# dash-robotics/perception

Hardware: AMD Instinct MI355X
Metric: frames/sec (640x480 D435 cloud, plane+cluster+ICP) (higher is better)
Workload: dtype f32

## Files before the change

perception_amd/csrc/common.hpp:

```cpp
#pragma once
#include <hip/hip_runtime.h>
#include <stdint.h>

#include "../../include/cuboid_hip.h"

namespace cd {

constexpr int WAVE = 64;
constexpr int BLOCK = 256;
constexpr int WAVES_PER_BLOCK = BLOCK / WAVE;
constexpr int ITEMS = 8;
constexpr int TILE = BLOCK * ITEMS;
constexpr int WAVE_SPAN = WAVE * ITEMS;
constexpr int RADIX_BITS = 8;
constexpr int RADIX = 1 << RADIX_BITS;
#ifndef CD_SORT_BLOCK
#define CD_SORT_BLOCK 1024
#endif
constexpr int SORT_BLOCK = CD_SORT_BLOCK;
constexpr int SORT_TILE = SORT_BLOCK * ITEMS;
constexpr int KICP = CD_MAX_CLUSTERS_PER_FRAME;
constexpr int FIX_SHIFT = 32;
constexpr int FIX_SHIFT_D2 = 36;
constexpr int RND_TABLE = 1 << 15;
// ... 23 lines not shown
    int32_t n_v;
    int32_t n_plane;
    int32_t n_o;
    int32_t n_k;
    int32_t n_hyp;
    int32_t sampler_exhausted;
    int32_t ksize[KICP];
    int32_t koff[KICP];
    float origin[3];
    int32_t n_cropped;
    int32_t cl_done;
    int32_t crop_overflow;
    int32_t scan_stalled;
    int32_t n_runs;
    int32_t digit_vary;
    int32_t pad_;
};

struct CropLimits {
    float zlo, zhi, xlo, xhi;
};

struct KeyPack {
    int32_t enabled;
    int32_t bi, bj;
    int32_t ilo, jlo, klo;
};

struct BBoxGate {
    double P[12];
    float rect[4];
// ... 240 lines not shown
```

perception_amd/csrc/cuboid_hip.hip:

```cpp
#include <algorithm>
#include <cstdio>
#include <cstdlib>
#include <cstring>
#include <memory>
#include <atomic>
#include <mutex>
#include <shared_mutex>
#include <condition_variable>
#include <random>
#include <vector>

#include "device_buffer.hpp"
#include "host_math.hpp"
#include "kernels.hpp"
#include "overlay_math.hpp"
#include "texture_math.hpp"

using namespace cd;

struct cd_streams {
    hipStream_t stream = nullptr, stream2 = nullptr, stream3 = nullptr;
    hipEvent_t ev[8] = {nullptr}, ev2[3] = {nullptr, nullptr, nullptr};
    ~cd_streams() {
        for (auto& e : ev2) if (e) hipEventDestroy(e);
// ... 5 lines not shown
struct cd_context : cd_streams {
    int device = 0;
    int N = 0, F = 0, T = 0;
    char err[512] = {0};
    DevBuf<char> d_in;
    DevBuf<uint16_t> d_depth;
    DevBuf<uint8_t> d_color;
    DevBuf<FrameState> d_fs;
    PinBuf<FrameState> h_fs;
    DevBuf<int> d_tileA, d_tileB, d_tileK, d_tileC;
    bool batch_zeroed = false;
    bool crop_two_pass = false;
    int icp_persist = 1;
    DevBuf<float4> d_cpt, d_vox, d_obj, d_src0, d_src;
    DevBuf<uint32_t> d_key[2], d_val[2], d_ghist;
    DevBuf<int> d_sstate;
    DevBuf<unsigned long long> d_tile64;
    bool crop_runs = true;
    DevBuf<int> d_ticket;
    DevBuf<int> d_rnd, d_valid, d_counts, d_active, d_have;
    PinBuf<int> h_valid, h_counts, h_active, h_have;
    DevBuf<float4> d_models, d_model;
    PinBuf<float4> h_model, h_models;
    DevBuf<unsigned long long> d_sums;
    PinBuf<unsigned long long> h_sums;
    DevBuf<int> d_plane_idx, d_head, d_next, d_parent, d_csize, d_rank, d_cand, d_sizes, d_label;
    DevBuf<float4> d_tpl, d_tlo, d_thi;
    DevBuf<float4> d_tplk, d_tlok, d_thik;
    DevBuf<IcpGrid> d_grid;
    DevBuf<unsigned short> d_kdmap;
// ... 10 lines not shown
    std::vector<IcpState> st_init;
    int force_stall = 0;
    int scan_retries = 0;
    int persist_gave_up = 0;
    int n_cu = 256;
    int icp_mode = 0;
    int icp_max_wg = 0;
    int icp_cpw = 0;
    bool fs_initialised = false;
    int icp_direct = 1;
    int mirror_reads = 1;
    int mirror_writes = 1;
    int cluster_cells = 1;
    int crop_direct = 1;
    int centroid_lanes = 1;
    bool voxel_runs = true;
    int icp_slots = 0;
    int icp_big_weight = 0;
    DevBuf<int> d_order; PinBuf<int> h_order;
    int tpl_cap = 0, tpl_used = 0;
    std::shared_ptr<const struct PreparedTemplate> tpl_prep[CD_MAX_TEMPLATES];
    int tpl_off[CD_MAX_TEMPLATES] = {0}, tpl_m[CD_MAX_TEMPLATES] = {0};
    bool tpl_gridded[CD_MAX_TEMPLATES] = {false};
    bool tpl_big[CD_MAX_TEMPLATES] = {false};
    DevBuf<IcpSuper> d_super;
    DevBuf<IcpLattice> d_lat;
    int tpl_faces[CD_MAX_TEMPLATES] = {0};
    int icp_lattice = 1;
    int zero_once = 1;
    int copy_kernels = 1;
// ... 281 lines not shown
        if (!over) break;
        if (std::getenv("CUBOID_DEBUG")) std::fprintf(stderr, "cuboid_hip: single-pass crop overflowed, redoing the batch in two passes\n");
        kp.enabled = 0;
        crop_runs = false;
        for (int f = 0; f < F; ++f) {
            FrameState& s = c->h_fs[f];
            std::memset(&s, 0, sizeof(s));
            for (int a = 0; a < 3; ++a) { s.mn[a] = 0xffffffffu; s.mx[a] = 0u; }
            }
    }
    int max_nc = 0, max_bits = 0;
    for (int f = 0; f < F; ++f) { max_nc = std::max(max_nc, c->h_fs[f].n_c); max_bits = std::max(max_bits, c->h_fs[f].key_bits); }
    const int Tc = std::max(1, (max_nc + TILE - 1) / TILE);
    const int Tsc = std::max(1, (max_nc + SORT_TILE - 1) / SORT_TILE);
    const int npass = (max_bits + RADIX_BITS - 1) / RADIX_BITS;
    int cur = 0;
    const bool by_runs = c->voxel_runs && npass > 0 && c->N <= (1 << 20);
    int Tc_runs = Tc;
    uint32_t* const key[2] = {c->d_key[0], c->d_key[1]}, * const val[2] = {c->d_val[0], c->d_val[1]};
    if (crop_runs) {
        int vary = 0, max_runs = 0;
        for (int f = 0; f < F; ++f) {
            if (c->h_fs[f].n_c > 0) vary |= c->h_fs[f].digit_vary;
            max_runs = std::max(max_runs, c->h_fs[f].n_runs);
        }
        int digits[4], nd = 0;
        for (int d = 0; d < 4; ++d) if ((vary >> d) & 1) digits[nd++] = d;
        const int Tsr = std::max(1, (max_runs + SORT_TILE - 1) / SORT_TILE);
        Tc_runs = std::max(1, (max_runs + TILE - 1) / TILE);
        LAUNCH(c, cur = launch_radix_scatter_runs(c->stream, key, val, c->N, F, Tsr, digits, nd, c->d_fs, c->d_ghist, c->d_sstate, c->d_ticket));
    } else if (by_runs)
        LAUNCH(c, cur = launch_radix_sort_runs(c->stream, key, val, c->N, F, T, Tsc, npass, c->d_fs, c->d_ghist, c->d_sstate, c->d_tileA, kp, c->d_ticket));
    else
        LAUNCH(c, cur = launch_radix_sort(c->stream, key, val, c->N, F, Tsc, npass, c->d_fs, c->d_ghist, c->d_sstate, kp, c->d_ticket));
    if (cur < 0) return fail(c, CD_ERR_DEVICE, "radix sort: the scan state could not be zeroed");
    const uint32_t* vin = c->d_val[cur];
    ZERO_FILL(c, c->d_tileC, sizeof(int) * (size_t)F * T);
    if (crop_runs || by_runs)
        LAUNCH(c, launch_voxel_centroid_runs(c->stream, c->d_key[cur], vin, crop_runs && direct_pts ? reinterpret_cast<const float4*>(d_in) : c->d_cpt, c->N, F, T, crop_runs ? Tc_runs : Tc,
                                             rgb_off >= 0 ? 1 : 0, c->d_fs, c->d_tileC, c->d_vox, c->d_ticket, c->centroid_lanes, crop_runs && direct_pts ? N : c->N));
    else
        LAUNCH(c, launch_voxel_centroid(c->stream, c->d_key[cur], vin, c->d_cpt, c->N, F, T, Tc, rgb_off >= 0 ? 1 : 0, c->d_fs, c->d_tileC, c->d_vox, c->d_ticket));
    if (rounds_out) *rounds_out = 0;
    return CD_OK;
}

int stage_plane(cd_context* c, int F, const cd_params* p, std::vector<int>& iterations, int* rounds_out, const float* axes = nullptr) {
    const int T = c->T;
    const bool mr = c->mirror_reads != 0;
    const float thr = hm::fold_ge(p->plane_distance_threshold);
    int max_nv = 0;
    for (int f = 0; f < F; ++f) max_nv = std::max(max_nv, c->h_fs[f].n_v);
    const int Tv = std::max(1, (max_nv + TILE - 1) / TILE);
// ... 859 lines not shown

int zero_batch_scratch(cd_context* c, int F) {
    ZeroRegions zr;
    zr.n = 0;
    zr.fs = c->mirror_writes && c->copy_kernels ? c->d_fs : nullptr;
    zr.nfs = F;
    c->fs_initialised = zr.fs != nullptr;
    auto add = [&](void* ptr, size_t bytes) { zr.ptr[zr.n] = (uint32_t*)ptr; zr.words[zr.n] = bytes / 4; ++zr.n; };
    const size_t FT = (size_t)F * c->T;
    add(c->d_ticket, sizeof(int) * (size_t)F * TICKET_PITCH);
    add(c->d_tileA, sizeof(int) * FT);
    add(c->d_tileB, sizeof(int) * FT);
    add(c->d_tileC, sizeof(int) * FT);
    add(c->d_tile64, sizeof(unsigned long long) * FT);
    add(c->d_ghist, sizeof(uint32_t) * (size_t)F * SORT_MAX_PASSES_HOST * RADIX);
    add(c->d_counts, sizeof(int) * (size_t)F * MAX_HYP);
    add(c->d_sums, sizeof(unsigned long long) * 10 * (size_t)F);
    add(c->d_tileK, sizeof(int) * FT * KICP);
    add(c->d_acc, sizeof(unsigned long long) * 48 * (size_t)c->cl_cap);
    add(c->d_accf, sizeof(unsigned long long) * ((size_t)c->cl_cap + 1));
    add(c->d_queue, sizeof(int) * 16);
    LAUNCH(c, launch_zero_regions(c->stream, zr));
    c->batch_zeroed = true;
    return CD_OK;
}

int batch_prologue(cd_context* c, int gate_source, const void* d_frames, int F, const DepthJob* dj) {
    if (gate_source == CD_BBOX_PER_FRAME) {
        std::memcpy(c->h_rects, c->frame_rects.data(), sizeof(int32_t) * 4 * (size_t)F);
        HIPCHK(c, xfer(c, c->d_rects, c->h_rects, sizeof(int32_t) * 4 * (size_t)F, hipMemcpyHostToDevice));
// ... 328 lines not shown
    switch (which) {
        case 0: return (int)sizeof(cd_params);
        case 1: return (int)sizeof(cd_cluster_result);
        case 2: return (int)sizeof(cd_frame_result);
        case 3: return (int)sizeof(cd_timing);
        case 4: return (int)sizeof(cd_depth_camera);
        case 5: return (int)sizeof(cd_color_gate_params);
        case 6: return (int)sizeof(cd_color_bbox);
        case 7: return (int)sizeof(cd_overlay_params);
        case 8: return (int)sizeof(cd_overlay_box);
        default: return -1;
    }
}

const char* cd_last_error(const cd_context* ctx) { return ctx ? ctx->err : "null context"; }

void cd_destroy(cd_context* c) {
    if (!c) return;
    hipSetDevice(c->device);
    for (hipStream_t q : {c->stream, c->stream2, c->stream3}) if (q) hipStreamSynchronize(q);
    delete c;
}

int cd_create(int device_id, int max_points, int max_frames, cd_context** out) {
    if (!out) return CD_ERR_INVALID_ARG;
    *out = nullptr;
    if (max_points <= 0 || max_frames <= 0) return CD_ERR_INVALID_ARG;
    int ndev = 0;
    if (hipGetDeviceCount(&ndev) != hipSuccess || ndev <= 0 || device_id < 0 || device_id >= ndev) return CD_ERR_DEVICE;
    if (hipSetDevice(device_id) != hipSuccess) return CD_ERR_DEVICE;
// ... 4 lines not shown
    c->F = max_frames;
    c->T = (max_points + TILE - 1) / TILE;
    const size_t N = (size_t)c->N, F = (size_t)c->F, T = (size_t)c->T, FN = F * N;
    if (const char* m = std::getenv("CUBOID_ICP_LOWPRIO")) c->icp_lowprio = std::atoi(m);
    int prio_least = 0, prio_greatest = 0;
    if (hipDeviceGetStreamPriorityRange(&prio_least, &prio_greatest) != hipSuccess) prio_least = prio_greatest = 0;
    bool ok = hipStreamCreateWithPriority(&c->stream, hipStreamNonBlocking, 0) == hipSuccess;
    for (auto& e : c->ev) ok = ok && hipEventCreate(&e) == hipSuccess;
    ok = ok && ALLOC(d_fs, F) && ALLOC(h_fs, F);
    ok = ok && ALLOC(d_tileA, F * T) && ALLOC(d_tileB, F * T) && ALLOC(d_tileK, F * KICP * T) && ALLOC(d_tileC, F * T);
    ok = ok && ALLOC(d_cpt, FN) && ALLOC(d_vox, FN) && ALLOC(d_obj, FN);
    ok = ok && ALLOC(d_src0, FN) && ALLOC(d_src, FN);
    for (int k = 0; k < 2; ++k) ok = ok && ALLOC(d_key[k], FN) && ALLOC(d_val[k], FN);
    ok = ok && ALLOC(d_ghist, F * SORT_MAX_PASSES_HOST * RADIX);
    ok = ok && ALLOC(d_sstate, (size_t)SORT_MAX_PASSES_HOST * F * RADIX * ((N + SORT_TILE - 1) / SORT_TILE));
    ok = ok && ALLOC(d_tile64, F * T);
    ok = ok && ALLOC(d_ticket, (size_t)F * TICKET_PITCH) && hipMemset(c->d_ticket, 0, sizeof(int) * (size_t)F * TICKET_PITCH) == hipSuccess;
    ok = ok && ALLOC(d_rnd, (size_t)RND_TABLE);
    ok = ok && ALLOC(d_models, F * MAX_HYP) && ALLOC(d_valid, F * MAX_HYP) && ALLOC(d_counts, F * MAX_HYP);
    ok = ok && ALLOC(h_valid, F * MAX_HYP) && ALLOC(h_counts, F * MAX_HYP) && ALLOC(h_models, F * MAX_HYP);
    ok = ok && ALLOC(d_active, F) && ALLOC(h_active, F);
    ok = ok && ALLOC(d_model, F) && ALLOC(h_model, F);
    ok = ok && ALLOC(d_have, F) && ALLOC(h_have, F);
    ok = ok && ALLOC(d_sums, F * 10) && ALLOC(h_sums, F * 10);
    ok = ok && ALLOC(d_plane_idx, FN) && ALLOC(d_head, F * CELL_BUCKETS);
    ok = ok && ALLOC(d_next, FN) && ALLOC(d_parent, FN) && ALLOC(d_csize, FN);
    ok = ok && ALLOC(d_rank, FN) && ALLOC(d_cand, FN) && ALLOC(d_sizes, FN) && ALLOC(d_label, FN);
    c->tpl_cap = 1 << 18;
    ok = ok && ALLOC(d_tpl, (size_t)c->tpl_cap);
    ok = ok && ALLOC(d_super, (size_t)CD_MAX_TEMPLATES);
    ok = ok && ALLOC(d_lat, (size_t)CD_MAX_TEMPLATES);
// ... 17 lines not shown
    c->cl_cap = (int)ncl;
    c->work_cap = (int)(F * (N / 64 + KICP + 1));
    ok = ok && ALLOC(d_cl, ncl) && ALLOC(h_cl, ncl);
    ok = ok && ALLOC(d_order, ncl) && ALLOC(h_order, ncl);
    if (const char* m = std::getenv("CUBOID_ICP_MAX_WG")) c->icp_max_wg = std::max(0, std::atoi(m));
    if (const char* m = std::getenv("CUBOID_ICP_CPW")) c->icp_cpw = std::max(0, std::atoi(m));
    if (const char* m = std::getenv("CUBOID_ICP_SLOTS")) c->icp_slots = std::max(0, std::atoi(m));
    if (const char* m = std::getenv("CUBOID_ICP_DONATE")) c->icp_donate = std::atoi(m);
    if (const char* m = std::getenv("CUBOID_ICP_DON_IDLE")) c->don_idle = std::max(0, std::atoi(m));
    if (const char* m = std::getenv("CUBOID_ICP_DON_FAULT")) c->don_fault = std::atoi(m);
    if (const char* m = std::getenv("CUBOID_ICP_LATTICE")) c->icp_lattice = std::atoi(m);
    if (const char* m = std::getenv("CUBOID_COPY_KERNELS")) c->copy_kernels = std::atoi(m);
    if (const char* m = std::getenv("CUBOID_ZERO_ONCE")) c->zero_once = std::atoi(m);
    if (const char* m = std::getenv("CUBOID_LAT_SHAPE")) std::sscanf(m, "%d,%d,%d", &c->lat_shape[0], &c->lat_shape[1], &c->lat_shape[2]);
    if (const char* m = std::getenv("CUBOID_VOXEL_RUNS")) c->voxel_runs = std::atoi(m) != 0;
    if (const char* m = std::getenv("CUBOID_CENTROID_LANES")) c->centroid_lanes = std::atoi(m) != 0;
    if (const char* m = std::getenv("CUBOID_CROP_DIRECT")) c->crop_direct = std::atoi(m) != 0;
    if (const char* m = std::getenv("CUBOID_CLUSTER_CELLS")) c->cluster_cells = std::atoi(m) != 0;
    if (const char* m = std::getenv("CUBOID_MIRROR_WRITES")) c->mirror_writes = std::atoi(m) != 0;
    if (const char* m = std::getenv("CUBOID_MIRROR_READS")) c->mirror_reads = std::atoi(m) != 0;
    if (const char* m = std::getenv("CUBOID_ICP_DIRECT")) c->icp_direct = std::atoi(m) != 0;
    if (const char* m = std::getenv("CUBOID_ICP_BIG_WEIGHT")) c->icp_big_weight = std::max(0, std::atoi(m));
    if (const char* m = std::getenv("CUBOID_CROP_TWO_PASS")) c->crop_two_pass = std::atoi(m) != 0;
    if (const char* m = std::getenv("CUBOID_ICP_PERSIST")) c->icp_persist = std::atoi(m);
    if (const char* m = std::getenv("CUBOID_FORCE_SCAN_STALL")) c->force_stall = std::max(0, std::atoi(m));
    if (const char* m = std::getenv("CUBOID_CROP_RUNS")) c->crop_runs = std::atoi(m) != 0;
    if (const char* m = std::getenv("CUBOID_ICP_CONCURRENT")) c->icp_concurrent = std::max(0, std::atoi(m));
    if (const char* m = std::getenv("CUBOID_FRONT_CONCURRENT")) c->front_concurrent = std::max(0, std::atoi(m));
    if (const char* m = std::getenv("CUBOID_ICP_MODE")) c->icp_mode = !std::strcmp(m, "sliced") ? 1 : (!std::strcmp(m, "cluster") ? 2 : (!std::strcmp(m, "pipe") ? 3 : 0));
    ok = ok && ALLOC(d_work, (size_t)c->work_cap) && ALLOC(h_work, (size_t)c->work_cap);
// ... 1511 lines not shown
```

perception_amd/csrc/k_voxel.hip:

```cpp
#include "kernels.hpp"

namespace cd {

template <int R>
__device__ __forceinline__ void load_rows(const char* __restrict__ in, size_t stride, size_t fbase, int first, int N, int rgb_off,
                                          float (&x)[R], float (&y)[R], float (&z)[R], uint32_t (&rgb)[R]) {
    if (stride == 16 && rgb_off == 12) {
        float4 v[R];
#pragma unroll
        for (int j = 0; j < R; ++j) v[j] = *reinterpret_cast<const float4*>(in + (fbase + (size_t)min(first + j * WAVE, N - 1)) * 16);
#pragma unroll
        for (int j = 0; j < R; ++j) { x[j] = v[j].x; y[j] = v[j].y; z[j] = v[j].z; rgb[j] = __float_as_uint(v[j].w); }
    } else {
#pragma unroll
        for (int j = 0; j < R; ++j) {
            const char* p = in + (fbase + (size_t)min(first + j * WAVE, N - 1)) * stride;
            x[j] = *reinterpret_cast<const float*>(p);
            y[j] = *reinterpret_cast<const float*>(p + 4);
            z[j] = *reinterpret_cast<const float*>(p + 8);
            rgb[j] = rgb_off >= 0 ? *reinterpret_cast<const uint32_t*>(p + rgb_off) : 0u;
        }
    }
}

// ... 112 lines not shown
        const int hi = (int)floorf(__fmul_rn(mx[a], inv));
        s.min_b[a] = lo;
        s.div_b[a] = hi - lo + 1;
        cells *= (long long)(hi - lo + 1);
        if (cells > 2147483647ll) bad = true;
    }
    if (bad) { s.status = CD_ERR_LEAF_TOO_SMALL; s.n_c = 0; s.n_runs = 0; return; }
    int bits = 1;
    while (bits < 31 && (1ll << bits) < cells) ++bits;
    s.key_bits = bits;
}
__global__ void __launch_bounds__(WAVE) k_voxel_setup(FrameState* __restrict__ fs, float leaf, const uint32_t* __restrict__ ghist,
                                                      FrameState* __restrict__ mirror) {
    CD_FRONT_PRIO();
    const int f = blockIdx.x, lane = threadIdx.x;
    int vary = 0;
    if (ghist) {
        for (int d = 0; d < 4; ++d) {
            int bins = 0;
            for (int q = 0; q < RADIX / WAVE; ++q) bins += __popcll(__ballot(ghist[((size_t)f * 4 + d) * RADIX + q * WAVE + lane] != 0u));
            if (bins > 1) vary |= 1 << d;
        }
    }
    if (lane != 0) return;
    FrameState s = fs[f];
    if (ghist) s.digit_vary = vary;
    voxel_setup_frame(s, leaf);
    fs[f] = s;
    if (mirror) mirror[f] = s;
}

__global__ void __launch_bounds__(BLOCK) k_crop_compact(const char* __restrict__ in, size_t stride, int N, int pitch,
                                                        int rgb_off, CropLimits lim, int T, float leaf,
                                                        const FrameState* __restrict__ fs,
                                                        const int* __restrict__ tile_off, float4* __restrict__ cpt,
                                                        uint32_t* __restrict__ keys) {
    CD_FRONT_PRIO();
    __shared__ int s_cnt[WAVES_PER_BLOCK];
    const int f = blockIdx.y, tile = blockIdx.x, w = threadIdx.x >> 6, lane = threadIdx.x & 63;
    if (fs[f].n_c <= 0) return;
    const size_t fbase = (size_t)f * N;
// ... 501 lines not shown
            }
        }
        if (ql == 0) {
            const float c = (float)cnt;
            uint32_t packed = 0;
            if (rgb_on) {
                const int R = (int)__fdiv_rn(cr, c), G = (int)__fdiv_rn(cg, c), B = (int)__fdiv_rn(cb, c);
                packed = ((uint32_t)R << 16) | ((uint32_t)G << 8) | (uint32_t)B;
            }
            vox[fbase + out0 + h] = make_float4(__fdiv_rn(sx, c), __fdiv_rn(sy, c), __fdiv_rn(sz, c), __uint_as_float(packed));
        }
        h = hn; e0 = ne0; kk = nkk; rec = nrec; have = nhave;
    }
}

__global__ void __launch_bounds__(BLOCK) k_voxel_centroid_lanes(const uint32_t* __restrict__ keys,
                                                                const uint32_t* __restrict__ vals,
                                                                const float4* __restrict__ cpt, int N, int T, int Tact, int rgb_on,
                                                                FrameState* __restrict__ fs, int* __restrict__ state,
                                                                float4* __restrict__ vox, int* __restrict__ ticket, int pts_pitch) {
    CD_FRONT_PRIO();
    __shared__ int s_cnt[WAVES_PER_BLOCK];
    __shared__ int s_head[TILE];
    __shared__ int s_out0, s_ticket;
    const int F = gridDim.x / Tact;
    const int f = blockIdx.x % F, tile = take_ticket(ticket + f * TICKET_PITCH, Tact, &s_ticket), w = threadIdx.x >> 6, lane = threadIdx.x & 63;
    const int n = fs[f].n_runs;
    if (tile * TILE >= n) return;
    const size_t fbase = (size_t)f * N;
    const uint32_t* k = keys + fbase;
// ... 9 lines not shown
    __syncthreads();
    int pos = 0, nheads = 0;
    for (int q = 0; q < WAVES_PER_BLOCK; ++q) { if (q < w) pos += s_cnt[q]; nheads += s_cnt[q]; }
    if (threadIdx.x == 0) {
        const int excl = chained_scan(state + (size_t)f * T, 1, tile, nheads, &fs[f].scan_stalled);
        s_out0 = excl;
        if ((tile + 1) * TILE >= n) fs[f].n_v = excl + nheads;
    }
    const uint64_t lt = lanemask_lt();
#pragma unroll
    for (int j = 0; j < ITEMS; ++j) {
        if ((bal[j] >> lane) & 1ull) s_head[pos + __popcll(bal[j] & lt)] = base + j * WAVE + lane;
        pos += __popcll(bal[j]);
    }
    __syncthreads();
    const int out0 = s_out0;
    constexpr uint32_t START = (1u << 20) - 1u;
    for (int h0 = w * WAVE; h0 < nheads; h0 += BLOCK) {
        const int h = h0 + lane;
        bool alive = h < nheads;
        int e = 0, i = 0, cnt = 0;
        uint32_t key = 0, wk0 = 0, wk1 = 0, wk2 = 0, wk3 = 0, wv0 = 0, wv1 = 0, wv2 = 0, wv3 = 0;
        if (alive) {
            e = s_head[h];
            key = k[e];
            wk0 = key; wv0 = v[e];
            wk1 = wk2 = wk3 = ~key;
            if (e + 1 < n) { wk1 = k[e + 1]; wv1 = v[e + 1]; }
            if (e + 2 < n) { wk2 = k[e + 2]; wv2 = v[e + 2]; }
            if (e + 3 < n) { wk3 = k[e + 3]; wv3 = v[e + 3]; }
        }
        uint32_t nk0 = 0, nk1 = 0, nk2 = 0, nk3 = 0, nv0 = 0, nv1 = 0, nv2 = 0, nv3 = 0;
        float sx = 0.f, sy = 0.f, sz = 0.f;
        uint32_t ir = 0, ig = 0, ib = 0;
        while (ballot64(alive)) {
            const bool m0 = alive && wk0 == key, m1 = m0 && wk1 == key, m2 = m1 && wk2 == key, m3 = m2 && wk3 == key;
            const int l0 = m0 ? (int)(wv0 >> 20) : 0, l1 = m1 ? (int)(wv1 >> 20) : 0, l2 = m2 ? (int)(wv2 >> 20) : 0, l3 = m3 ? (int)(wv3 >> 20) : 0;
            const int c1 = l0, c2 = c1 + l1, c3 = c2 + l2, tot = c3 + l3;
            const int s0 = (int)(wv0 & START), s1 = (int)(wv1 & START) - c1, s2 = (int)(wv2 & START) - c2, s3 = (int)(wv3 & START) - c3;
            if (m3 && i == 0) {
                nk0 = nk1 = nk2 = nk3 = ~key;
                if (e + 4 < n) { nk0 = k[e + 4]; nv0 = v[e + 4]; }
                if (e + 5 < n) { nk1 = k[e + 5]; nv1 = v[e + 5]; }
                if (e + 6 < n) { nk2 = k[e + 6]; nv2 = v[e + 6]; }
                if (e + 7 < n) { nk3 = k[e + 7]; nv3 = v[e + 7]; }
            }
            const float4 z = make_float4(0.f, 0.f, 0.f, 0.f);
            float4 P[8];
#pragma unroll
            for (int t = 0; t < 8; ++t) {
                const int idx = i + t;
                const int off = idx >= c3 ? s3 : (idx >= c2 ? s2 : (idx >= c1 ? s1 : s0));
                P[t] = z;
                if (idx < tot && CD_IN_RANGE(off + idx >= 0 && off + idx < pts_pitch, 4u)) P[t] = pts[off + idx];
            }
#pragma unroll
            for (int t = 0; t < 8; ++t) {
                sx = __fadd_rn(sx, P[t].x); sy = __fadd_rn(sy, P[t].y); sz = __fadd_rn(sz, P[t].z);
                if (rgb_on) {
                    const uint32_t u = __float_as_uint(P[t].w);
                    ir = __builtin_amdgcn_udot4(u, 0x00010000u, ir, false);
                    ig = __builtin_amdgcn_udot4(u, 0x00000100u, ig, false);
                    ib = __builtin_amdgcn_udot4(u, 0x00000001u, ib, false);
                }
            }
            i += 8;
            if (alive && i >= tot) {
                cnt += tot;
                alive = m3 && nk0 == key;
                e += 4; i = 0;
                wk0 = nk0; wk1 = nk1; wk2 = nk2; wk3 = nk3; wv0 = nv0; wv1 = nv1; wv2 = nv2; wv3 = nv3;
            }
        }
        if (h < nheads) {
            float cr = (float)ir, cg = (float)ig, cb = (float)ib;
            if (rgb_on && cnt > 65536) {
                cr = cg = cb = 0.f;
                for (int ee = s_head[h]; ee < n && k[ee] == key; ++ee) {
                    const uint32_t r = v[ee];
                    const int s0 = (int)(r & START), ln = (int)(r >> 20);
                    for (int i = 0; i < ln; ++i) {
                        const uint32_t u = __float_as_uint(pts[s0 + i].w);
                        cr += (float)((u >> 16) & 0xff); cg += (float)((u >> 8) & 0xff); cb += (float)(u & 0xff);
                    }
                }
            }
            const float c = (float)cnt;
            uint32_t packed = 0;
            if (rgb_on) {
                const int R = (int)__fdiv_rn(cr, c), G = (int)__fdiv_rn(cg, c), B = (int)__fdiv_rn(cb, c);
                packed = ((uint32_t)R << 16) | ((uint32_t)G << 8) | (uint32_t)B;
            }
            vox[fbase + out0 + h] = make_float4(__fdiv_rn(sx, c), __fdiv_rn(sy, c), __fdiv_rn(sz, c), __uint_as_float(packed));
        }
    }
}

void launch_crop_count(hipStream_t s, const void* in, size_t stride, int N, int F, int rgb_off, CropLimits lim, int T,
                       FrameState* fs, int* tile_cnt) {
    const int Tin = (N + TILE - 1) / TILE;
    hipLaunchKernelGGL(k_crop_count, dim3(Tin, F), dim3(BLOCK), 0, s, (const char*)in, stride, N, rgb_off, lim, T, fs, tile_cnt);
}
void launch_scan_tiles(hipStream_t s, int* counts, int rows, int T, int* totals, int total_pitch) {
    const ScanJob j{counts, totals, nullptr};
    hipLaunchKernelGGL(k_scan_tiles, dim3(rows, 1), dim3(BLOCK), 0, s, j, j, T, total_pitch);
}
void launch_scan_tiles2(hipStream_t s, const ScanJob& a, const ScanJob& b, int rows, int T, int total_pitch) {
    hipLaunchKernelGGL(k_scan_tiles, dim3(rows, 2), dim3(BLOCK), 0, s, a, b, T, total_pitch);
}
void launch_voxel_setup(hipStream_t s, FrameState* fs, int F, float leaf, const uint32_t* ghist, FrameState* mirror) {
// ... 23 lines not shown
                           leaf, kp, fs, state, cpt, rkeys, rvals, ghist, ticket);
}
void launch_voxel_centroid(hipStream_t s, const uint32_t* keys, const uint32_t* vals, const float4* cpt, int N, int F,
                           int T, int Tact, int rgb_on, FrameState* fs, int* state, float4* vox, int* ticket) {
    hipLaunchKernelGGL(k_voxel_centroid, dim3(Tact * F), dim3(BLOCK), 0, s, keys, vals, cpt, N, T, Tact, rgb_on, fs, state, vox, ticket);
}
void launch_voxel_centroid_runs(hipStream_t s, const uint32_t* keys, const uint32_t* vals, const float4* cpt, int N, int F,
                                int T, int Tact, int rgb_on, FrameState* fs, int* state, float4* vox, int* ticket, int lanes, int pts_pitch) {
    if (lanes) {
        hipLaunchKernelGGL(k_voxel_centroid_lanes, dim3(Tact * F), dim3(BLOCK), 0, s, keys, vals, cpt, N, T, Tact, rgb_on, fs, state, vox, ticket, pts_pitch);
        return;
    }
    hipLaunchKernelGGL(k_voxel_centroid_runs, dim3(Tact * F), dim3(BLOCK), 0, s, keys, vals, cpt, N, T, Tact, rgb_on, fs, state, vox, ticket, pts_pitch);
}

}
```

perception_amd/csrc/kernels.hpp:

```cpp
#pragma once
#include "common.hpp"

namespace cd {

void launch_crop_count(hipStream_t s, const void* in, size_t stride, int N, int F, int rgb_off, CropLimits lim, int T,
                       FrameState* fs, int* tile_cnt);
struct ScanJob { int* counts; int* totals; int* mirror; };
void launch_scan_tiles(hipStream_t s, int* counts, int rows, int T, int* totals, int total_pitch);
void launch_scan_tiles2(hipStream_t s, const ScanJob& a, const ScanJob& b, int rows, int T, int total_pitch);
void launch_voxel_setup(hipStream_t s, FrameState* fs, int F, float leaf, const uint32_t* ghist, FrameState* mirror);
void launch_crop_fused(hipStream_t s, const void* in, size_t stride, int N, int pitch, int F, int rgb_off, CropLimits lim,
                       int T, float leaf, KeyPack kp, FrameState* fs, int* state, float4* cpt, uint32_t* keys, int* ticket);
void launch_crop_runs(hipStream_t s, const void* in, size_t stride, int N, int pitch, int F, int rgb_off, CropLimits lim,
                      int T, float leaf, KeyPack kp, FrameState* fs, unsigned long long* state, float4* cpt, uint32_t* rkeys,
                      uint32_t* rvals, uint32_t* ghist, int* ticket, int direct);
void launch_crop_compact(hipStream_t s, const void* in, size_t stride, int N, int pitch, int F, int rgb_off, CropLimits lim,
                         int T, float leaf, const FrameState* fs, const int* tile_off, float4* cpt, uint32_t* keys);
void launch_voxel_centroid(hipStream_t s, const uint32_t* keys, const uint32_t* vals, const float4* cpt, int N, int F,
                           int T, int Tact, int rgb_on, FrameState* fs, int* state, float4* vox, int* ticket);
void launch_voxel_centroid_runs(hipStream_t s, const uint32_t* keys, const uint32_t* vals, const float4* cpt, int N, int F,
                                int T, int Tact, int rgb_on, FrameState* fs, int* state, float4* vox, int* ticket, int lanes, int pts_pitch);

void launch_mark_indices(hipStream_t s, const int* idx, int m, int n, int* flag);
struct ZeroRegions { int n; uint32_t* ptr[16]; size_t words[16]; FrameState* fs; int nfs; };
void launch_zero_regions(hipStream_t s, const ZeroRegions& r);
struct CopySeg { uint32_t* dst; const uint32_t* src; size_t dpitch_w, spitch_w; int width_w, rows; };
struct CopyList { int n; CopySeg seg[8]; };
void launch_copy_list(hipStream_t s, const CopyList& L);
void launch_copy_rows(hipStream_t s, void* dst, size_t dpitch, const void* src, size_t spitch, size_t width, int rows);
void launch_passthrough_mark(hipStream_t s, const void* in, size_t stride, int n, int field_off, double lo, double hi, int negative, int* flag);
void launch_select_unmarked(hipStream_t s, const int* flag, int n, int* state, FrameState* fs, int* out, int* ticket);
void launch_gather_records(hipStream_t s, const void* in, int words, const int* idx, int m, void* out);
void launch_pack_records(hipStream_t s, const float4* pts, int m, int words, int rgb_word, uint32_t pad3, void* out);

constexpr int SORT_MAX_PASSES_HOST = 4;
int launch_radix_sort(hipStream_t s, uint32_t* const key[2], uint32_t* const val[2], int N, int F, int Tact, int npass,
// ... 102 lines not shown
```

Before: 184,500.

## Sort voxel keys by top digit only and finish low digits per bucket in LDS

The global radix scatter now runs a single pass on the top varying digit. A new bucket kernel, one block per top-digit bucket, sorts the remaining low digits in shared memory and computes voxel centroids directly, replacing the extra global scatter passes and the separate centroid kernel. Voxel setup records the largest top-digit bucket so the host can pick a block size or fall back to the old path. The cost is a larger shared-memory footprint per block, a fixed grid of RADIX blocks per frame, and more complex code. The change also adds debug accessors.

```diff
diff --git a/perception_amd/csrc/common.hpp b/perception_amd/csrc/common.hpp
--- a/perception_amd/csrc/common.hpp
+++ b/perception_amd/csrc/common.hpp
@@ -61,7 +61,7 @@
     int32_t scan_stalled;
     int32_t n_runs;
     int32_t digit_vary;
-    int32_t pad_;
+    int32_t max_bucket;
 };
 
 struct CropLimits {
diff --git a/perception_amd/csrc/cuboid_hip.hip b/perception_amd/csrc/cuboid_hip.hip
--- a/perception_amd/csrc/cuboid_hip.hip
+++ b/perception_amd/csrc/cuboid_hip.hip
@@ -43,6 +43,7 @@
     int icp_persist = 1;
     DevBuf<float4> d_cpt, d_vox, d_obj, d_src0, d_src;
     DevBuf<uint32_t> d_key[2], d_val[2], d_ghist;
+    DevBuf<int> d_bstate;
     DevBuf<int> d_sstate;
     DevBuf<unsigned long long> d_tile64;
     bool crop_runs = true;
@@ -83,6 +84,8 @@
     int cluster_cells = 1;
     int crop_direct = 1;
     int centroid_lanes = 1;
+    bool voxel_buckets = true;
+    int dbg_voxel[4] = {0, 0, 0, 0};
     bool voxel_runs = true;
     int icp_slots = 0;
     int icp_big_weight = 0;
@@ -394,7 +397,9 @@
     const int Tc = std::max(1, (max_nc + TILE - 1) / TILE);
     const int Tsc = std::max(1, (max_nc + SORT_TILE - 1) / SORT_TILE);
     const int npass = (max_bits + RADIX_BITS - 1) / RADIX_BITS;
-    int cur = 0;
+    int cur = 0, bucket_arg[3] = {0, 0, 0};
+    bool buckets = false;
+    c->dbg_voxel[0] = c->dbg_voxel[1] = c->dbg_voxel[2] = c->dbg_voxel[3] = 0;
     const bool by_runs = c->voxel_runs && npass > 0 && c->N <= (1 << 20);
     int Tc_runs = Tc;
     uint32_t* const key[2] = {c->d_key[0], c->d_key[1]}, * const val[2] = {c->d_val[0], c->d_val[1]};
@@ -408,15 +413,32 @@
         for (int d = 0; d < 4; ++d) if ((vary >> d) & 1) digits[nd++] = d;
         const int Tsr = std::max(1, (max_runs + SORT_TILE - 1) / SORT_TILE);
         Tc_runs = std::max(1, (max_runs + TILE - 1) / TILE);
-        LAUNCH(c, cur = launch_radix_scatter_runs(c->stream, key, val, c->N, F, Tsr, digits, nd, c->d_fs, c->d_ghist, c->d_sstate, c->d_ticket));
+        int bucket_max = 0;
+        const int top = nd > 0 ? digits[nd - 1] : 0;
+        for (int f = 0; f < F; ++f) {
+            const FrameState& s = c->h_fs[f];
+            if (s.n_c <= 0 || s.n_runs <= 0) continue;
+            bucket_max = std::max(bucket_max, ((s.digit_vary >> top) & 1) ? s.max_bucket : s.n_runs);
+        }
+        buckets = c->voxel_buckets && c->centroid_lanes && c->crop_direct && nd >= 2 && bucket_max <= voxel_buckets_cap();
+        c->dbg_voxel[0] = buckets ? 1 : 0; c->dbg_voxel[1] = top; c->dbg_voxel[2] = bucket_max; c->dbg_voxel[3] = vary;
+        if (buckets) {
+            ZERO_FILL(c, c->d_bstate, sizeof(int) * (size_t)F * RADIX);
+            LAUNCH(c, cur = launch_radix_scatter_runs(c->stream, key, val, c->N, F, Tsr, &top, 1, c->d_fs, c->d_ghist, c->d_sstate, c->d_ticket));
+        } else
+            LAUNCH(c, cur = launch_radix_scatter_runs(c->stream, key, val, c->N, F, Tsr, digits, nd, c->d_fs, c->d_ghist, c->d_sstate, c->d_ticket));
+        bucket_arg[0] = top; bucket_arg[1] = vary & ((1 << top) - 1); bucket_arg[2] = bucket_max;
     } else if (by_runs)
         LAUNCH(c, cur = launch_radix_sort_runs(c->stream, key, val, c->N, F, T, Tsc, npass, c->d_fs, c->d_ghist, c->d_sstate, c->d_tileA, kp, c->d_ticket));
     else
         LAUNCH(c, cur = launch_radix_sort(c->stream, key, val, c->N, F, Tsc, npass, c->d_fs, c->d_ghist, c->d_sstate, kp, c->d_ticket));
     if (cur < 0) return fail(c, CD_ERR_DEVICE, "radix sort: the scan state could not be zeroed");
     const uint32_t* vin = c->d_val[cur];
-    ZERO_FILL(c, c->d_tileC, sizeof(int) * (size_t)F * T);
-    if (crop_runs || by_runs)
+    if (!buckets) ZERO_FILL(c, c->d_tileC, sizeof(int) * (size_t)F * T);
+    if (buckets)
+        LAUNCH(c, launch_voxel_buckets(c->stream, c->d_key[cur], vin, direct_pts ? reinterpret_cast<const float4*>(d_in) : c->d_cpt, c->N, F, bucket_arg[0], bucket_arg[1],
+                                       bucket_arg[2], rgb_off >= 0 ? 1 : 0, c->d_fs, c->d_ghist, c->d_bstate, c->d_vox, c->d_ticket, direct_pts ? N : c->N));
+    else if (crop_runs || by_runs)
         LAUNCH(c, launch_voxel_centroid_runs(c->stream, c->d_key[cur], vin, crop_runs && direct_pts ? reinterpret_cast<const float4*>(d_in) : c->d_cpt, c->N, F, T, crop_runs ? Tc_runs : Tc,
                                              rgb_off >= 0 ? 1 : 0, c->d_fs, c->d_tileC, c->d_vox, c->d_ticket, c->centroid_lanes, crop_runs && direct_pts ? N : c->N));
     else
@@ -1306,6 +1328,7 @@
     add(c->d_tileC, sizeof(int) * FT);
     add(c->d_tile64, sizeof(unsigned long long) * FT);
     add(c->d_ghist, sizeof(uint32_t) * (size_t)F * SORT_MAX_PASSES_HOST * RADIX);
+    add(c->d_bstate, sizeof(int) * (size_t)F * RADIX);
     add(c->d_counts, sizeof(int) * (size_t)F * MAX_HYP);
     add(c->d_sums, sizeof(unsigned long long) * 10 * (size_t)F);
     add(c->d_tileK, sizeof(int) * FT * KICP);
@@ -1664,6 +1687,18 @@
 }
 
 const char* cd_last_error(const cd_context* ctx) { return ctx ? ctx->err : "null context"; }
+
+extern "C" int cd_debug_voxel_path(const cd_context* c, int32_t* out) {
+    if (!c || !out) return CD_ERR_INVALID_ARG;
+    for (int q = 0; q < 4; ++q) out[q] = c->dbg_voxel[q];
+    return CD_OK;
+}
+extern "C" int cd_debug_voxel_hist(cd_context* c, int frame, int digit, uint32_t* out) {
+    if (!c || !out || frame < 0 || frame >= c->F || digit < 0 || digit >= SORT_MAX_PASSES_HOST) return CD_ERR_INVALID_ARG;
+    if (hipSetDevice(c->device) != hipSuccess || hipStreamSynchronize(c->stream) != hipSuccess) return CD_ERR_DEVICE;
+    const uint32_t* src = c->d_ghist.get() + ((size_t)frame * SORT_MAX_PASSES_HOST + digit) * RADIX;
+    return hipMemcpy(out, src, sizeof(uint32_t) * RADIX, hipMemcpyDeviceToHost) == hipSuccess ? CD_OK : CD_ERR_DEVICE;
+}
 
 void cd_destroy(cd_context* c) {
     if (!c) return;
@@ -1698,7 +1733,7 @@
     for (int k = 0; k < 2; ++k) ok = ok && ALLOC(d_key[k], FN) && ALLOC(d_val[k], FN);
     ok = ok && ALLOC(d_ghist, F * SORT_MAX_PASSES_HOST * RADIX);
     ok = ok && ALLOC(d_sstate, (size_t)SORT_MAX_PASSES_HOST * F * RADIX * ((N + SORT_TILE - 1) / SORT_TILE));
-    ok = ok && ALLOC(d_tile64, F * T);
+    ok = ok && ALLOC(d_tile64, F * T) && ALLOC(d_bstate, F * RADIX);
     ok = ok && ALLOC(d_ticket, (size_t)F * TICKET_PITCH) && hipMemset(c->d_ticket, 0, sizeof(int) * (size_t)F * TICKET_PITCH) == hipSuccess;
     ok = ok && ALLOC(d_rnd, (size_t)RND_TABLE);
     ok = ok && ALLOC(d_models, F * MAX_HYP) && ALLOC(d_valid, F * MAX_HYP) && ALLOC(d_counts, F * MAX_HYP);
@@ -1746,6 +1781,7 @@
     if (const char* m = std::getenv("CUBOID_ZERO_ONCE")) c->zero_once = std::atoi(m);
     if (const char* m = std::getenv("CUBOID_LAT_SHAPE")) std::sscanf(m, "%d,%d,%d", &c->lat_shape[0], &c->lat_shape[1], &c->lat_shape[2]);
     if (const char* m = std::getenv("CUBOID_VOXEL_RUNS")) c->voxel_runs = std::atoi(m) != 0;
+    if (const char* m = std::getenv("CUBOID_VOXEL_BUCKETS")) c->voxel_buckets = std::atoi(m) != 0;
     if (const char* m = std::getenv("CUBOID_CENTROID_LANES")) c->centroid_lanes = std::atoi(m) != 0;
     if (const char* m = std::getenv("CUBOID_CROP_DIRECT")) c->crop_direct = std::atoi(m) != 0;
     if (const char* m = std::getenv("CUBOID_CLUSTER_CELLS")) c->cluster_cells = std::atoi(m) != 0;
diff --git a/perception_amd/csrc/k_voxel.hip b/perception_amd/csrc/k_voxel.hip
--- a/perception_amd/csrc/k_voxel.hip
+++ b/perception_amd/csrc/k_voxel.hip
@@ -150,17 +150,26 @@
                                                       FrameState* __restrict__ mirror) {
     CD_FRONT_PRIO();
     const int f = blockIdx.x, lane = threadIdx.x;
-    int vary = 0;
+    int vary = 0, top_max = 0;
     if (ghist) {
         for (int d = 0; d < 4; ++d) {
-            int bins = 0;
-            for (int q = 0; q < RADIX / WAVE; ++q) bins += __popcll(__ballot(ghist[((size_t)f * 4 + d) * RADIX + q * WAVE + lane] != 0u));
-            if (bins > 1) vary |= 1 << d;
+            int bins = 0, mx = 0;
+            for (int q = 0; q < RADIX / WAVE; ++q) {
+                const uint32_t cnt = ghist[((size_t)f * 4 + d) * RADIX + q * WAVE + lane];
+                bins += __popcll(__ballot(cnt != 0u));
+                mx = max(mx, (int)cnt);
+            }
+            if (bins > 1) {
+                vary |= 1 << d;
+#pragma unroll
+                for (int o = 32; o > 0; o >>= 1) mx = max(mx, __shfl_xor(mx, o, 64));
+                top_max = mx;
+            }
         }
     }
     if (lane != 0) return;
     FrameState s = fs[f];
-    if (ghist) s.digit_vary = vary;
+    if (ghist) { s.digit_vary = vary; s.max_bucket = top_max; }
     voxel_setup_frame(s, leaf);
     fs[f] = s;
     if (mirror) mirror[f] = s;
@@ -692,6 +701,92 @@
     }
 }
 
+template <typename H>
+__device__ __forceinline__ void centroid_lanes_sum(const uint32_t* k, const uint32_t* v, int n, const H* s_head, int nheads, int w,
+                                                   int nthreads, const float4* __restrict__ pts, int pts_pitch, int rgb_on,
+                                                   float4* __restrict__ out, int out_room) {
+    const int lane = threadIdx.x & 63;
+    constexpr uint32_t START = (1u << 20) - 1u;
+    for (int h0 = w * WAVE; h0 < nheads; h0 += nthreads) {
+        const int h = h0 + lane;
+        bool alive = h < nheads;
+        int e = 0, i = 0, cnt = 0;
+        uint32_t key = 0, wk0 = 0, wk1 = 0, wk2 = 0, wk3 = 0, wv0 = 0, wv1 = 0, wv2 = 0, wv3 = 0;
+        if (alive) {
+            e = s_head[h];
+            key = k[e];
+            wk0 = key; wv0 = v[e];
+            wk1 = wk2 = wk3 = ~key;
+            if (e + 1 < n) { wk1 = k[e + 1]; wv1 = v[e + 1]; }
+            if (e + 2 < n) { wk2 = k[e + 2]; wv2 = v[e + 2]; }
+            if (e + 3 < n) { wk3 = k[e + 3]; wv3 = v[e + 3]; }
+        }
+        uint32_t nk0 = 0, nk1 = 0, nk2 = 0, nk3 = 0, nv0 = 0, nv1 = 0, nv2 = 0, nv3 = 0;
+        float sx = 0.f, sy = 0.f, sz = 0.f;
+        uint32_t ir = 0, ig = 0, ib = 0;
+        while (ballot64(alive)) {
+            const bool m0 = alive && wk0 == key, m1 = m0 && wk1 == key, m2 = m1 && wk2 == key, m3 = m2 && wk3 == key;
+            const int l0 = m0 ? (int)(wv0 >> 20) : 0, l1 = m1 ? (int)(wv1 >> 20) : 0, l2 = m2 ? (int)(wv2 >> 20) : 0, l3 = m3 ? (int)(wv3 >> 20) : 0;
+            const int c1 = l0, c2 = c1 + l1, c3 = c2 + l2, tot = c3 + l3;
+            const int s0 = (int)(wv0 & START), s1 = (int)(wv1 & START) - c1, s2 = (int)(wv2 & START) - c2, s3 = (int)(wv3 & START) - c3;
+            if (m3 && i == 0) {
+                nk0 = nk1 = nk2 = nk3 = ~key;
+                if (e + 4 < n) { nk0 = k[e + 4]; nv0 = v[e + 4]; }
+                if (e + 5 < n) { nk1 = k[e + 5]; nv1 = v[e + 5]; }
+                if (e + 6 < n) { nk2 = k[e + 6]; nv2 = v[e + 6]; }
+                if (e + 7 < n) { nk3 = k[e + 7]; nv3 = v[e + 7]; }
+            }
+            const float4 z = make_float4(0.f, 0.f, 0.f, 0.f);
+            float4 P[8];
+#pragma unroll
+            for (int t = 0; t < 8; ++t) {
+                const int idx = i + t;
+                const int off = idx >= c3 ? s3 : (idx >= c2 ? s2 : (idx >= c1 ? s1 : s0));
+                P[t] = z;
+                if (idx < tot && CD_IN_RANGE(off + idx >= 0 && off + idx < pts_pitch, 4u)) P[t] = pts[off + idx];
+            }
+#pragma unroll
+            for (int t = 0; t < 8; ++t) {
+                sx = __fadd_rn(sx, P[t].x); sy = __fadd_rn(sy, P[t].y); sz = __fadd_rn(sz, P[t].z);
+                if (rgb_on) {
+                    const uint32_t u = __float_as_uint(P[t].w);
+                    ir = __builtin_amdgcn_udot4(u, 0x00010000u, ir, false);
+                    ig = __builtin_amdgcn_udot4(u, 0x00000100u, ig, false);
+                    ib = __builtin_amdgcn_udot4(u, 0x00000001u, ib, false);
+                }
+            }
+            i += 8;
+            if (alive && i >= tot) {
+                cnt += tot;
+                alive = m3 && nk0 == key;
+                e += 4; i = 0;
+                wk0 = nk0; wk1 = nk1; wk2 = nk2; wk3 = nk3; wv0 = nv0; wv1 = nv1; wv2 = nv2; wv3 = nv3;
+            }
+        }
+        if (h < nheads) {
+            float cr = (float)ir, cg = (float)ig, cb = (float)ib;
+            if (rgb_on && cnt > 65536) {
+                cr = cg = cb = 0.f;
+                for (int ee = s_head[h]; ee < n && k[ee] == key; ++ee) {
+                    const uint32_t r = v[ee];
+                    const int s0 = (int)(r & START), ln = (int)(r >> 20);
+                    for (int i = 0; i < ln; ++i) {
+                        const uint32_t u = __float_as_uint(pts[s0 + i].w);
+                        cr += (float)((u >> 16) & 0xff); cg += (float)((u >> 8) & 0xff); cb += (float)(u & 0xff);
+                    }
+                }
+            }
+            const float c = (float)cnt;
+            uint32_t packed = 0;
+            if (rgb_on) {
+                const int R = (int)__fdiv_rn(cr, c), G = (int)__fdiv_rn(cg, c), B = (int)__fdiv_rn(cb, c);
+                packed = ((uint32_t)R << 16) | ((uint32_t)G << 8) | (uint32_t)B;
+            }
+            if (CD_IN_RANGE(h < out_room, 6u)) out[h] = make_float4(__fdiv_rn(sx, c), __fdiv_rn(sy, c), __fdiv_rn(sz, c), __uint_as_float(packed));
+        }
+    }
+}
+
 __global__ void __launch_bounds__(BLOCK) k_voxel_centroid_lanes(const uint32_t* __restrict__ keys,
                                                                 const uint32_t* __restrict__ vals,
                                                                 const float4* __restrict__ cpt, int N, int T, int Tact, int rgb_on,
@@ -731,86 +826,180 @@
         pos += __popcll(bal[j]);
     }
     __syncthreads();
+    centroid_lanes_sum(k, v, n, s_head, nheads, w, BLOCK, pts, pts_pitch, rgb_on, vox + fbase + s_out0, N - s_out0);
+}
+
+template <int NT, int ROWS>
+__global__ void __launch_bounds__(NT) k_voxel_buckets(const uint32_t* __restrict__ keys, const uint32_t* __restrict__ vals,
+                                                      const float4* __restrict__ cpt, int N, int top, int low_mask, int rgb_on,
+                                                      FrameState* __restrict__ fs, const uint32_t* __restrict__ ghist,
+                                                      int* __restrict__ state, float4* __restrict__ vox, int* __restrict__ ticket,
+                                                      int pts_pitch) {
+    constexpr int NW = NT / WAVE, CAP = NT * ROWS;
+    static_assert(NT >= RADIX && CAP <= 65535, "one thread per bin; 16-bit bin counts and head positions");
+    CD_FRONT_PRIO();
+    __shared__ uint32_t s_k[CAP], s_v[CAP];
+    __shared__ unsigned short s_head[CAP];
+    __shared__ unsigned short s_wh[NW][RADIX];
+    __shared__ uint32_t s_bstart[RADIX];
+    __shared__ uint32_t s_ws[RADIX / WAVE];
+    __shared__ int s_part[RADIX / WAVE], s_cnt[NW];
+    __shared__ int s_n, s_out0, s_ticket;
+    const int F = gridDim.x / RADIX;
+    const int f = blockIdx.x % F, b = take_ticket(ticket + f * TICKET_PITCH, RADIX, &s_ticket), w = threadIdx.x >> 6, lane = threadIdx.x & 63;
+    const int nr = fs[f].n_runs;
+    if (nr <= 0) return;
+    if (threadIdx.x < RADIX) {
+        const int c = (int)ghist[((size_t)f * 4 + top) * RADIX + threadIdx.x];
+        const int below = wave_sum_i32((int)threadIdx.x < b ? c : 0);
+        if (lane == 0) s_part[w] = below;
+        if ((int)threadIdx.x == b) s_n = c;
+    }
+    __syncthreads();
+    int start = 0;
+    for (int q = 0; q < RADIX / WAVE; ++q) start += s_part[q];
+    int n = s_n;
+    if (n > CAP || start + n > nr) {
+        if (threadIdx.x == 0) fs[f].scan_stalled = 1;
+        n = 0;
+    }
+    if (n == 0) {
+        if (threadIdx.x == 0) {
+            const int excl = chained_scan(state + (size_t)f * RADIX, 1, b, 0, &fs[f].scan_stalled);
+            if (b == RADIX - 1) fs[f].n_v = excl;
+        }
+        return;
+    }
+    const size_t fbase = (size_t)f * N;
+    const int rpw = (n + NT - 1) / NT;
+    const int e0 = w * rpw * WAVE + lane;
+    const uint64_t lt = lanemask_lt();
+    uint32_t key[ROWS], val[ROWS], rank[ROWS];
+#pragma unroll
+    for (int j = 0; j < ROWS; ++j) {
+        const int e = e0 + j * WAVE;
+        const bool valid = j < rpw && e < n && CD_IN_RANGE(start + e < nr, 7u);
+        key[j] = valid ? keys[fbase + start + e] : 0xffffffffu;
+        val[j] = valid ? vals[fbase + start + e] : 0u;
+    }
+    bool in_regs = true;
+    for (int dg = 0; dg < top; ++dg) {
+        if (!((low_mask >> dg) & 1)) continue;
+        const int shift = dg * RADIX_BITS;
+        for (int q = threadIdx.x; q < NW * RADIX; q += NT) (&s_wh[0][0])[q] = 0;
+        if (!in_regs) {
+#pragma unroll
+            for (int j = 0; j < ROWS; ++j) {
+                const int e = e0 + j * WAVE;
+                const bool valid = j < rpw && e < n;
+                key[j] = valid ? s_k[e] : 0xffffffffu;
+                val[j] = valid ? s_v[e] : 0u;
+            }
+        }
+        __syncthreads();
+#pragma unroll
+        for (int j = 0; j < ROWS; ++j) {
+            if (j < rpw) {
+                const int e = e0 + j * WAVE;
+                const bool valid = e < n;
+                const uint32_t d = (key[j] >> shift) & (RADIX - 1);
+                uint32_t dl = 0u, dh = 0u;
+#pragma unroll
+                for (int bit = 0; bit < RADIX_BITS; ++bit) {
+                    const int y = (int)(d << (31 - bit)) >> 31;
+                    const uint64_t m = __ballot(y < 0);
+                    dl |= (uint32_t)m ^ (uint32_t)y;
+                    dh |= (uint32_t)(m >> 32) ^ (uint32_t)y;
+                }
+                const uint64_t peers = ~(((uint64_t)dh << 32) | dl) & __ballot(valid);
+                uint32_t bin_base = 0;
+                if (valid) bin_base = s_wh[w][d];
+                if (valid && (peers >> lane) == 1ull) s_wh[w][d] = (unsigned short)(bin_base + (uint32_t)__popcll(peers));
+                rank[j] = bin_base + (uint32_t)__popcll(peers & lt);
+            }
+        }
+        __syncthreads();
+        if (threadIdx.x < RADIX) {
+            const int d = threadIdx.x;
+            uint32_t run = 0;
+#pragma unroll
+            for (int q = 0; q < NW; ++q) {
+                const uint32_t c = s_wh[q][d];
+                s_wh[q][d] = (unsigned short)run;
+                run += c;
+            }
+            uint32_t inc = run;
+#pragma unroll
+            for (int o = 1; o < 64; o <<= 1) {
+                const uint32_t u = __shfl_up(inc, o, 64);
+                if (lane >= o) inc += u;
+            }
+            if (lane == 63) s_ws[w] = inc;
+            s_bstart[d] = inc - run;
+        }
+        __syncthreads();
+        if (threadIdx.x < RADIX) {
+            uint32_t add = 0;
+            for (int q = 0; q < w; ++q) add += s_ws[q];
+            s_bstart[threadIdx.x] += add;
+        }
+        __syncthreads();
+#pragma unroll
+        for (int j = 0; j < ROWS; ++j) {
+            const int e = e0 + j * WAVE;
+            if (j < rpw && e < n) {
+                const uint32_t d = (key[j] >> shift) & (RADIX - 1);
+                const uint32_t lp = s_bstart[d] + s_wh[w][d] + rank[j];
+                if (CD_IN_RANGE(lp < (uint32_t)n, 8u)) {
+                    s_k[lp] = key[j];
+                    s_v[lp] = val[j];
+                }
+            }
+        }
+        __syncthreads();
+        in_regs = false;
+    }
+    if (in_regs) {
+#pragma unroll
+        for (int j = 0; j < ROWS; ++j) {
+            const int e = e0 + j * WAVE;
+            if (j < rpw && e < n) { s_k[e] = key[j]; s_v[e] = val[j]; }
+        }
+        __syncthreads();
+    }
+    const uint32_t* k = s_k;
+    const uint32_t* v = s_v;
+    uint64_t bal[ROWS];
+    int wtot = 0;
+#pragma unroll
+    for (int j = 0; j < ROWS; ++j) {
+        const int e = e0 + j * WAVE;
+        const bool in = j < rpw && e < n;
+        const uint32_t me = in ? k[e] : 0u, left = in && e > 0 ? k[e - 1] : 0u;
+        bal[j] = ballot64(in && (e == 0 || me != left));
+        wtot += __popcll(bal[j]);
+    }
+    if (lane == 0) s_cnt[w] = wtot;
+    __syncthreads();
+    int pos = 0, nheads = 0;
+    for (int q = 0; q < NW; ++q) { if (q < w) pos += s_cnt[q]; nheads += s_cnt[q]; }
+    if (threadIdx.x == 0) {
+        const int excl = chained_scan(state + (size_t)f * RADIX, 1, b, nheads, &fs[f].scan_stalled);
+        s_out0 = excl;
+        if (b == RADIX - 1) fs[f].n_v = excl + nheads;
+    }
+#pragma unroll
+    for (int j = 0; j < ROWS; ++j) {
+        if ((bal[j] >> lane) & 1ull) {
+            const int hp = pos + __popcll(bal[j] & lt);
+            if (CD_IN_RANGE(hp < n, 9u)) s_head[hp] = (unsigned short)(e0 + j * WAVE);
+        }
+        pos += __popcll(bal[j]);
+    }
+    __syncthreads();
+    const float4* pts = cpt + (size_t)f * pts_pitch;
     const int out0 = s_out0;
-    constexpr uint32_t START = (1u << 20) - 1u;
-    for (int h0 = w * WAVE; h0 < nheads; h0 += BLOCK) {
-        const int h = h0 + lane;
-        bool alive = h < nheads;
-        int e = 0, i = 0, cnt = 0;
-        uint32_t key = 0, wk0 = 0, wk1 = 0, wk2 = 0, wk3 = 0, wv0 = 0, wv1 = 0, wv2 = 0, wv3 = 0;
-        if (alive) {
-            e = s_head[h];
-            key = k[e];
-            wk0 = key; wv0 = v[e];
-            wk1 = wk2 = wk3 = ~key;
-            if (e + 1 < n) { wk1 = k[e + 1]; wv1 = v[e + 1]; }
-            if (e + 2 < n) { wk2 = k[e + 2]; wv2 = v[e + 2]; }
-            if (e + 3 < n) { wk3 = k[e + 3]; wv3 = v[e + 3]; }
-        }
-        uint32_t nk0 = 0, nk1 = 0, nk2 = 0, nk3 = 0, nv0 = 0, nv1 = 0, nv2 = 0, nv3 = 0;
-        float sx = 0.f, sy = 0.f, sz = 0.f;
-        uint32_t ir = 0, ig = 0, ib = 0;
-        while (ballot64(alive)) {
-            const bool m0 = alive && wk0 == key, m1 = m0 && wk1 == key, m2 = m1 && wk2 == key, m3 = m2 && wk3 == key;
-            const int l0 = m0 ? (int)(wv0 >> 20) : 0, l1 = m1 ? (int)(wv1 >> 20) : 0, l2 = m2 ? (int)(wv2 >> 20) : 0, l3 = m3 ? (int)(wv3 >> 20) : 0;
-            const int c1 = l0, c2 = c1 + l1, c3 = c2 + l2, tot = c3 + l3;
-            const int s0 = (int)(wv0 & START), s1 = (int)(wv1 & START) - c1, s2 = (int)(wv2 & START) - c2, s3 = (int)(wv3 & START) - c3;
-            if (m3 && i == 0) {
-                nk0 = nk1 = nk2 = nk3 = ~key;
-                if (e + 4 < n) { nk0 = k[e + 4]; nv0 = v[e + 4]; }
-                if (e + 5 < n) { nk1 = k[e + 5]; nv1 = v[e + 5]; }
-                if (e + 6 < n) { nk2 = k[e + 6]; nv2 = v[e + 6]; }
-                if (e + 7 < n) { nk3 = k[e + 7]; nv3 = v[e + 7]; }
-            }
-            const float4 z = make_float4(0.f, 0.f, 0.f, 0.f);
-            float4 P[8];
-#pragma unroll
-            for (int t = 0; t < 8; ++t) {
-                const int idx = i + t;
-                const int off = idx >= c3 ? s3 : (idx >= c2 ? s2 : (idx >= c1 ? s1 : s0));
-                P[t] = z;
-                if (idx < tot && CD_IN_RANGE(off + idx >= 0 && off + idx < pts_pitch, 4u)) P[t] = pts[off + idx];
-            }
-#pragma unroll
-            for (int t = 0; t < 8; ++t) {
-                sx = __fadd_rn(sx, P[t].x); sy = __fadd_rn(sy, P[t].y); sz = __fadd_rn(sz, P[t].z);
-                if (rgb_on) {
-                    const uint32_t u = __float_as_uint(P[t].w);
-                    ir = __builtin_amdgcn_udot4(u, 0x00010000u, ir, false);
-                    ig = __builtin_amdgcn_udot4(u, 0x00000100u, ig, false);
-                    ib = __builtin_amdgcn_udot4(u, 0x00000001u, ib, false);
-                }
-            }
-            i += 8;
-            if (alive && i >= tot) {
-                cnt += tot;
-                alive = m3 && nk0 == key;
-                e += 4; i = 0;
-                wk0 = nk0; wk1 = nk1; wk2 = nk2; wk3 = nk3; wv0 = nv0; wv1 = nv1; wv2 = nv2; wv3 = nv3;
-            }
-        }
-        if (h < nheads) {
-            float cr = (float)ir, cg = (float)ig, cb = (float)ib;
-            if (rgb_on && cnt > 65536) {
-                cr = cg = cb = 0.f;
-                for (int ee = s_head[h]; ee < n && k[ee] == key; ++ee) {
-                    const uint32_t r = v[ee];
-                    const int s0 = (int)(r & START), ln = (int)(r >> 20);
-                    for (int i = 0; i < ln; ++i) {
-                        const uint32_t u = __float_as_uint(pts[s0 + i].w);
-                        cr += (float)((u >> 16) & 0xff); cg += (float)((u >> 8) & 0xff); cb += (float)(u & 0xff);
-                    }
-                }
-            }
-            const float c = (float)cnt;
-            uint32_t packed = 0;
-            if (rgb_on) {
-                const int R = (int)__fdiv_rn(cr, c), G = (int)__fdiv_rn(cg, c), B = (int)__fdiv_rn(cb, c);
-                packed = ((uint32_t)R << 16) | ((uint32_t)G << 8) | (uint32_t)B;
-            }
-            vox[fbase + out0 + h] = make_float4(__fdiv_rn(sx, c), __fdiv_rn(sy, c), __fdiv_rn(sz, c), __uint_as_float(packed));
-        }
-    }
+    centroid_lanes_sum(k, v, n, s_head, nheads, w, NT, pts, pts_pitch, rgb_on, vox + fbase + out0, N - out0);
 }
 
 void launch_crop_count(hipStream_t s, const void* in, size_t stride, int N, int F, int rgb_off, CropLimits lim, int T,
@@ -864,4 +1053,15 @@
     hipLaunchKernelGGL(k_voxel_centroid_runs, dim3(Tact * F), dim3(BLOCK), 0, s, keys, vals, cpt, N, T, Tact, rgb_on, fs, state, vox, ticket, pts_pitch);
 }
 
-}
+int voxel_buckets_cap() { return 1024 * 8; }
+void launch_voxel_buckets(hipStream_t s, const uint32_t* keys, const uint32_t* vals, const float4* cpt, int N, int F, int top, int low_mask,
+                          int bucket_max, int rgb_on, FrameState* fs, const uint32_t* ghist, int* state, float4* vox, int* ticket, int pts_pitch) {
+    if (bucket_max <= 256 * 10)
+        hipLaunchKernelGGL((k_voxel_buckets<256, 10>), dim3(RADIX * F), dim3(256), 0, s, keys, vals, cpt, N, top, low_mask, rgb_on, fs, ghist, state, vox, ticket, pts_pitch);
+    else if (bucket_max <= 512 * 10)
+        hipLaunchKernelGGL((k_voxel_buckets<512, 10>), dim3(RADIX * F), dim3(512), 0, s, keys, vals, cpt, N, top, low_mask, rgb_on, fs, ghist, state, vox, ticket, pts_pitch);
+    else
+        hipLaunchKernelGGL((k_voxel_buckets<1024, 8>), dim3(RADIX * F), dim3(1024), 0, s, keys, vals, cpt, N, top, low_mask, rgb_on, fs, ghist, state, vox, ticket, pts_pitch);
+}
+
+}
diff --git a/perception_amd/csrc/kernels.hpp b/perception_amd/csrc/kernels.hpp
--- a/perception_amd/csrc/kernels.hpp
+++ b/perception_amd/csrc/kernels.hpp
@@ -20,6 +20,9 @@
                            int T, int Tact, int rgb_on, FrameState* fs, int* state, float4* vox, int* ticket);
 void launch_voxel_centroid_runs(hipStream_t s, const uint32_t* keys, const uint32_t* vals, const float4* cpt, int N, int F,
                                 int T, int Tact, int rgb_on, FrameState* fs, int* state, float4* vox, int* ticket, int lanes, int pts_pitch);
+int voxel_buckets_cap();
+void launch_voxel_buckets(hipStream_t s, const uint32_t* keys, const uint32_t* vals, const float4* cpt, int N, int F, int top, int low_mask,
+                          int bucket_max, int rgb_on, FrameState* fs, const uint32_t* ghist, int* state, float4* vox, int* ticket, int pts_pitch);
 
 void launch_mark_indices(hipStream_t s, const int* idx, int m, int n, int* flag);
 struct ZeroRegions { int n; uint32_t* ptr[16]; size_t words[16]; FrameState* fs; int nfs; };
```

After: 175,700. 0.953x the previous value.
